# FRBNY-DSGE/SMC.jl

Measured on AMD Instinct MI355X. Metric: particle-stages/sec, higher is better.
Workload: dtype f64; 1 GPU; gauss10_isotropic_adaptive_phi_n100k (BASELINE config 2); n_parts_total=100000, n_parts_per_gpu=100000, n_para=10, n_phi=300, resampling=systematic, n_blocks=1, n_mh_steps=1, launch_mode=direct, history=True, parallelism=particles sharded x1

## Files before the change

smc.jl_amd/csrc/prof2.hpp:

```cpp
#pragma once

static int prof2_report(smcmi_handle *h0, const Geo2 &g0, int seg_launches) {
    {
        long long pr[128], gt[64], gp[64];
        HIP_TRY(hipMemcpy(pr, h0->e2->d_prof + PROF2_SEG0, 64 * sizeof(long long), hipMemcpyDeviceToHost));
        HIP_TRY(hipMemcpy(gt, h0->e2->d_prof + PROF2_GATH, sizeof(gt), hipMemcpyDeviceToHost));
        HIP_TRY(hipMemcpy(gp, h0->e2->d_prof + PROF2_GPOLL, sizeof(gp), hipMemcpyDeviceToHost));
        if (seg_launches > 0) {
            fprintf(stderr, "[smcmi3] stage %d worker 0 ticks: correction + row %lld | wait for the totals %lld | decision + proposal %lld | MH steps %lld | mutation row %lld | next stage's draws %lld | wait for the totals %lld | begin %lld | stage %lld\n",
                    h0->e2->prof_stage, pr[2] - pr[1], pr[3] - pr[2], pr[4] - pr[3], pr[5] - pr[4], pr[6] - pr[5], pr[7] - pr[6], pr[8] - pr[7], pr[9] - pr[8], pr[9] - pr[1]);
            fprintf(stderr, "[smcmi3]   stamps relative to the stage's first:");
            for (int q = 1; q <= 9; ++q) fprintf(stderr, " [%d] %lld", q, pr[q] - pr[1]);
            fprintf(stderr, "\n");
            {
                long long sp[10];
                HIP_TRY(hipMemcpy(sp, h0->e2->d_prof + PROF2_SEL, sizeof(sp), hipMemcpyDeviceToHost));
                if (sp[9]) fprintf(stderr, "[smcmi3]   selection inside the segment (wall clock, us): particle stored %.2f | chunk offsets %.2f | scan + cum %.2f | stores acknowledged %.2f | hand-over %.2f | chunk ends %.2f | search %.2f | rows gathered %.2f | moment row %.2f | hand-over %.2f\n",
                                   0.0, (sp[1] - sp[0]) * 0.01, (sp[2] - sp[1]) * 0.01, (sp[3] - sp[2]) * 0.01, (sp[4] - sp[3]) * 0.01, (sp[5] - sp[4]) * 0.01, (sp[6] - sp[5]) * 0.01, (sp[7] - sp[6]) * 0.01, (sp[8] - sp[7]) * 0.01, (sp[9] - sp[8]) * 0.01);
            }
            fprintf(stderr, "[smcmi3]   decision + proposal: totals -> covariance, shuffle %lld | block matrices %lld | Cholesky + log det %lld | rest %lld\n",
                    pr[30] - pr[3], pr[31] - pr[30], pr[32] - pr[31], pr[4] - pr[32]);
        }
        if (seg_launches > 0) {
            const int Wk = g0.Vl * g0.nb2;
            std::vector<long long> ws(4 * (size_t)Wk);
            HIP_TRY(hipMemcpy(ws.data(), h0->e2->d_prof + PROF2_WORK, sizeof(long long) * ws.size(), hipMemcpyDeviceToHost));
            for (int kind = 0; kind < 2; ++kind) {
                long long p_min = 0, p_max = 0, s_min = 0, s_max = 0;
                for (int b = 0; b < Wk; ++b) {
                    const long long pb = ws[4 * b + 2 * kind], sb = ws[4 * b + 2 * kind + 1];
                    if (!b || pb < p_min) p_min = pb;
                    if (!b || pb > p_max) p_max = pb;
                    if (!b || sb < s_min) s_min = sb;
                    if (!b || sb > s_max) s_max = sb;
                }
                fprintf(stderr, "[smcmi3] hand-over %d (%s rows): rows published over %.2f us (worker 0 at +%.2f); totals seen by the first worker +%.2f, the last +%.2f, worker 0 +%.2f after the first row\n",
                        kind, kind ? "mutation" : "correction", (p_max - p_min) * 0.01, (ws[2 * kind] - p_min) * 0.01, (s_min - p_min) * 0.01, (s_max - p_min) * 0.01, (ws[2 * kind + 1] - p_min) * 0.01);
                for (int v = 0; v < g0.Vl; ++v) {
                    long long lastrow = 0;
                    for (int b = v; b < Wk; b += g0.Vl) lastrow = std::max(lastrow, ws[4 * b + 2 * kind]);
                    fprintf(stderr, "[smcmi3]   gatherer %d: its last row +%.2f | first words seen +%.2f | %lld sweep(s) done +%.2f | totals posted +%.2f (started waiting at +%.2f)\n", v, (lastrow - p_min) * 0.01,
                            (gp[4 * v + 2 * kind] - p_min) * 0.01, gp[4 * v + 2 * kind + 1],
                            (gt[6 * v + 3 * kind + 1] - p_min) * 0.01, (gt[6 * v + 3 * kind + 2] - p_min) * 0.01, (gt[6 * v + 3 * kind] - p_min) * 0.01);
                }
            }
        }
        if (!g0.direct && !g0.inker && !g0.wide) {
            std::vector<long long> cs(3 * PROF2_BLOCKS);
            HIP_TRY(hipMemcpy(cs.data(), h0->e2->d_prof + PROF2_CENSUS, sizeof(long long) * cs.size(), hipMemcpyDeviceToHost));
            long long t_min = 0, t_max = 0, sum = 0;
            int nbk = 0;
            std::map<long long, std::vector<std::pair<long long, int>>> per_cu;
            for (int b = 0; b < PROF2_BLOCKS; ++b) {
                const long long t_a = cs[3 * b], t_b = cs[3 * b + 1];
                if (!t_a || !t_b) continue;
                if (!nbk || t_a < t_min) t_min = t_a;
                if (!nbk || t_b > t_max) t_max = t_b;
                sum += t_b - t_a;
                ++nbk;
                per_cu[cs[3 * b + 2]].push_back({t_a, +1});
                per_cu[cs[3 * b + 2]].push_back({t_b, -1});
            }
            int hist[9] = {0, 0, 0, 0, 0, 0, 0, 0, 0};
            for (auto &kv : per_cu) {
                std::sort(kv.second.begin(), kv.second.end());
                int cur = 0, mx = 0;
                for (auto &ev : kv.second) { cur += ev.second; mx = std::max(mx, cur); }
                hist[std::min(mx, 8)] += 1;
            }
            if (nbk) {
                fprintf(stderr, "[smcmi2] K2b census: %d blocks on %d CUs, first start -> last end %.2f us, mean block %.2f us, mean residency %.1f blocks; CUs by the most blocks they held at once:", nbk,
                        (int)per_cu.size(), (t_max - t_min) * 0.01, sum * 0.01 / nbk, (double)sum / (double)std::max<long long>(1, t_max - t_min));
                for (int k = 1; k <= 8; ++k) if (hist[k]) fprintf(stderr, " %d x %d", hist[k], k);
                int st_h[8] = {0, 0, 0, 0, 0, 0, 0, 0}, du_h[8] = {0, 0, 0, 0, 0, 0, 0, 0};
                const double st_e[7] = {1, 2, 5, 10, 15, 20, 25}, du_e[7] = {8, 12, 16, 20, 24, 28, 32};
                for (int b = 0; b < PROF2_BLOCKS; ++b) {
                    if (!cs[3 * b] || !cs[3 * b + 1]) continue;
                    const double st = (cs[3 * b] - t_min) * 0.01, du = (cs[3 * b + 1] - cs[3 * b]) * 0.01;
                    int k = 0; while (k < 7 && st >= st_e[k]) ++k; st_h[k] += 1;
                    k = 0; while (k < 7 && du >= du_e[k]) ++k; du_h[k] += 1;
                }
                fprintf(stderr, "\n[smcmi2]   started at <1 <2 <5 <10 <15 <20 <25 >=25 us:");
                for (int k = 0; k < 8; ++k) fprintf(stderr, " %d", st_h[k]);
                fprintf(stderr, "; ran <8 <12 <16 <20 <24 <28 <32 >=32 us:");
                for (int k = 0; k < 8; ++k) fprintf(stderr, " %d", du_h[k]);
                fprintf(stderr, "\n");
            }
        }
        HIP_TRY(hipMemcpy(pr, h0->e2->d_prof + PROF2_K1, 128 * sizeof(long long), hipMemcpyDeviceToHost));
        for (int blk = 0; blk < 2; ++blk) {
            fprintf(stderr, "[smcmi2] K1 %s block ticks:", blk ? "mid" : "0");
            for (int q = 1; q <= 5; ++q) fprintf(stderr, " %lld", pr[blk * 32 + q] - pr[blk * 32 + q - 1]);
            fprintf(stderr, "  total %lld\n[smcmi2] K2 %s block ticks:", pr[blk * 32 + 5] - pr[blk * 32], blk ? "mid" : "0");
            for (int q = 1; q <= 11; ++q) fprintf(stderr, " %lld", pr[64 + blk * 32 + q] - pr[64 + blk * 32 + q - 1]);
            fprintf(stderr, "  total %lld\n", pr[64 + blk * 32 + 10] - pr[64 + blk * 32]);
        }
    }
    return 0;
}
```

smc.jl_amd/csrc/stage2.hpp:

```cpp
#pragma once
#include "kernels.hpp"

namespace smcmi {

constexpr int RMAX_IDX = 32;
constexpr int T1 = 512;

constexpr int PROF2_BLOCKS = 4096;
constexpr int PROF2_K1 = 0, PROF2_K2 = 64, PROF2_CENSUS = 128, PROF2_SEG0 = PROF2_CENSUS + 3 * PROF2_BLOCKS, PROF2_SEL = PROF2_SEG0 + 64,
              PROF2_GATH = PROF2_SEL + 16, PROF2_GPOLL = PROF2_GATH + 64, PROF2_WORK = PROF2_GPOLL + 64, PROF2_WORDS = PROF2_WORK + 4 * 256;
#define K2_STAMP(prof, slot)                                                                                                   \
    do {                                                                                                                      \
        if ((prof) != nullptr && threadIdx.x == 0 && (blockIdx.x == 0 || blockIdx.x == gridDim.x / 2)) {                       \
            unsigned long long tt_;                                                                                           \
            asm volatile("s_waitcnt vmcnt(0) lgkmcnt(0)\n\ts_memtime %0\n\ts_waitcnt lgkmcnt(0)" : "=s"(tt_)::"memory");       \
            (prof)[(blockIdx.x == 0 ? 0 : 32) + (slot)] = (long long)tt_;                                                      \
        }                                                                                                                     \
    } while (0)

#define K3_STAMP_ANY(prof, slot)                                                                                               \
    do {                                                                                                                      \
        if ((prof) != nullptr && threadIdx.x == 0) {                                                                           \
            unsigned long long tt_;                                                                                           \
            asm volatile("s_waitcnt vmcnt(0) lgkmcnt(0)\n\ts_memtime %0\n\ts_waitcnt lgkmcnt(0)" : "=s"(tt_)::"memory");       \
            (prof)[(slot)] = (long long)tt_;                                                                                   \
        }                                                                                                                     \
    } while (0)

struct Geo2 {
    long long N, n, nv;
    int V, Vl, v0;
    int nb1, nb2, nbg;
    long long per1, perg;
    int t2;
    int direct;
    int inker;
    int wide;
};

struct Rows2 {
    const double *p;
    int nvs, nr, ld;
    const unsigned long long *mb;
    unsigned tag;
    unsigned long long *to;
};

constexpr int MB_LD = 72;
constexpr int MB_TABLE_WORDS = V2_MAXV * MB_LD * 2;
constexpr int MB_KINDS = 2;
constexpr int MB_WORDS = MB_KINDS * 2 * MB_TABLE_WORDS;
constexpr long long MB_TIMEOUT_TICKS_DEFAULT = 1000000000ll;
constexpr int MB_FLAG_WORDS = 2;
constexpr int MB_SEG_OFF = MB_WORDS + MB_FLAG_WORDS;
constexpr int MB_SEG_KIND_WORDS = V2_MAXV * MB_LD * 2;
constexpr int MB_SEG_COPY_WORDS = 2 * MB_SEG_KIND_WORDS;
constexpr int MB_ALLOC_WORDS = MB_SEG_OFF + 2 * MB_SEG_COPY_WORDS;
constexpr long long MB_SEL_CS_WORDS = 1024 * 2, MB_SEL_T_WORDS = V2_MAXV * 2 * 2, MB_SEL_GM_WORDS = V2_MAXV * 72 * 2;
constexpr long long MB_SEL_OFF = MB_ALLOC_WORDS, MB_SEL_TABLE_WORDS = MB_SEL_CS_WORDS + MB_SEL_T_WORDS + MB_SEL_GM_WORDS;
__device__ inline void mb_store(unsigned long long *w, double v, unsigned tag) {
    const unsigned long long b = (unsigned long long)__double_as_longlong(v);
    __hip_atomic_store(w, ((unsigned long long)tag << 32) | (b & 0xffffffffull), __ATOMIC_RELAXED, __HIP_MEMORY_SCOPE_SYSTEM);
    __hip_atomic_store(w + 1, ((unsigned long long)tag << 32) | (b >> 32), __ATOMIC_RELAXED, __HIP_MEMORY_SCOPE_SYSTEM);
}
__device__ inline double mb_load(const unsigned long long *w, unsigned tag, unsigned long long *to) {
    unsigned long long a = __hip_atomic_load(w, __ATOMIC_RELAXED, __HIP_MEMORY_SCOPE_SYSTEM);
    unsigned long long b = __hip_atomic_load(w + 1, __ATOMIC_RELAXED, __HIP_MEMORY_SCOPE_SYSTEM);
    if ((unsigned)(a >> 32) != tag || (unsigned)(b >> 32) != tag) {
        const long long t0 = wall_clock64();
        do {
            if (__hip_atomic_load(to, __ATOMIC_RELAXED, __HIP_MEMORY_SCOPE_AGENT)) return __builtin_nan("");
            __builtin_amdgcn_s_sleep(2);
            a = __hip_atomic_load(w, __ATOMIC_RELAXED, __HIP_MEMORY_SCOPE_SYSTEM);
            b = __hip_atomic_load(w + 1, __ATOMIC_RELAXED, __HIP_MEMORY_SCOPE_SYSTEM);
            if (wall_clock64() - t0 > (long long)__hip_atomic_load(to + 1, __ATOMIC_RELAXED, __HIP_MEMORY_SCOPE_AGENT)) {
                __hip_atomic_store(to, 1ull, __ATOMIC_RELAXED, __HIP_MEMORY_SCOPE_AGENT);
                return __builtin_nan("");
            }
        } while ((unsigned)(a >> 32) != tag || (unsigned)(b >> 32) != tag);
    }
    return __longlong_as_double((long long)((b << 32) | (a & 0xffffffffull)));
}
template <int M, int T>
__device__ inline void mbox_totals(const Rows2 &R, double *vt, double *tot, int max_idx) {
    for (int idx = threadIdx.x; idx < R.nvs * M; idx += T) {
        const int v = idx / M, k = idx % M;
        vt[idx] = mb_load(R.mb + ((long long)v * MB_LD + k) * 2, R.tag, R.to);
    }
    __syncthreads();
    for (int k = threadIdx.x; k < M; k += T) {
        const bool mx = k == max_idx;
        double t = mx ? -__builtin_inf() : 0.0;
        for (int v = 0; v < R.nvs; ++v) { const double x = vt[v * M + k]; t = mx ? fmax(t, x) : t + x; }
        tot[k] = t;
    }
    __syncthreads();
}

struct Begin2 {
    int stage, final, spec, j;
    double phi_prev, phi_n, phi_prop, ess_bar, gprime, pred_delta;
    double accept;
    double e_shift, e_center;
    double cfac;
    double e_seen;
};
struct Post2 {
    int stage, j, resampled_last, do_resample, resamples, fold_valid;
    double phi_n, phi_prop, ess, sumw, sumw2, logz, c, accept, e_center, e_shift;
    double e_seen;
// ... 1182 lines not shown
    const double *wt;
    double *rows_mut;
    Tail2 tail;
    double *hist_W;
    long long hist_ld;
    Records rec;
    int debug;
    long long *prof;
};

__device__ inline void post2(int n, const Begin2 &bg, const Post2 &po, const RunParams &rp, double s1, double s2, double ess, int rs, Post2 *out) {
    const double a = bg.accept;
    Post2 p = po;
    p.stage = n; p.j = bg.j; p.resampled_last = rs; p.do_resample = rs; p.resamples = po.resamples + rs; p.fold_valid = 1;
    p.phi_n = bg.phi_n; p.phi_prop = bg.phi_prop; p.ess = ess; p.sumw = s1; p.sumw2 = s2;
    const double dlz = (bg.phi_n - bg.phi_prev) * bg.e_shift;
    p.logz = po.logz + (log(s1 / (double)rp.n_parts) + dlz);
    p.c = po.c * bg.cfac;
    p.accept = a; p.e_center = bg.e_center; p.e_shift = bg.e_shift; p.e_seen = bg.e_seen;
    *out = p;
}

struct Prop2 {
    double *covl, *A, *mean;
    int *bfree, *bptr, *fi;
    double *Lraw, *logdet, *mub, *sdd, *sdn;
    int *ball, *loff;
    double *Ls;
};
template <int DB>
__device__ inline bool chol_full(double (&r)[12], int lane) {
    double q[DB];
#pragma unroll
    for (int k = 0; k < DB; ++k) q[k] = r[k];
    const bool ok = chol_rows_in_regs<DB, true, true>(q, DB, lane);
#pragma unroll
    for (int k = 0; k < DB; ++k) r[k] = q[k];
    return ok;
}
__device__ inline bool chol_full_dispatch(double (&r)[12], int d, int lane) {
    switch (d) {
    case 2: return chol_full<2>(r, lane); case 3: return chol_full<3>(r, lane); case 4: return chol_full<4>(r, lane);
    case 5: return chol_full<5>(r, lane); case 6: return chol_full<6>(r, lane); case 7: return chol_full<7>(r, lane);
    case 8: return chol_full<8>(r, lane); case 9: return chol_full<9>(r, lane); default: return chol_full<10>(r, lane);
    }
}

__device__ inline int shuffle_partner(unsigned long long seed, unsigned stage, int i0, int nf) {
    int jx = 0;
    if (i0 >= 1 && i0 < nf) {
        double ua, ub;
        uniform_pair(seed, 0ull, stage, rng_tag(P_BLK, (unsigned)i0, 0), ua, ub);
        jx = (int)(ua * (double)(i0 + 1));
        if (jx > i0) jx = i0;
    }
    return jx;
}

__device__ inline void shuffle_trace(int jx, int lane, int nf, int nb, int *bfree, int *bptr) {
    int pos = lane;
    for (int i = 1; i < nf; ++i) {
        const int ji = __shfl(jx, i, 64);
        pos = pos == i ? ji : (pos == ji ? i : pos);
    }
    if (lane < nf) bfree[lane] = pos;
    const int sub = (nf + nb - 1) / nb;
    if (lane < nb) bptr[lane] = lane * sub;
    if (lane == nb) bptr[nb] = nf;
}

constexpr int A1F_SHUF = 1;
constexpr int A1F_NOMIX = 2;
constexpr int A1F_LOGDET = 4;
constexpr int A1F_LS = 8;
#ifndef SMCMI_A1FAST
#define SMCMI_A1FAST (A1F_SHUF | A1F_NOMIX | A1F_LOGDET | A1F_LS)
#endif
constexpr int A1F_BOUNDS = 16;
constexpr int A1F_PRIOR = 32;
#ifndef SMCMI_A1TARGET
#define SMCMI_A1TARGET (A1F_BOUNDS | A1F_PRIOR)
#endif
static_assert(A1F_BOUNDS == (TGT_BOUNDS << 4) && A1F_PRIOR == (TGT_PRIOR << 4), "k2_mh_steps hands FAST >> 4 to mh_step");

template <int CHM = 12, int FAST = 0>
__device__ inline bool proposal2(const double *T, const double *shift, int d, int nf, int nb, double c, unsigned long long seed,
                                 unsigned stage, const Prop2 &P, int *s_fail, int TT, int jx_pre, long long *prof = nullptr, long long *prof_any = nullptr) {
    const int t = threadIdx.x, da = d + 1;
    const double sw = T[0];
    if (t == 0) *s_fail = 0;
    for (int e = t; e < d * d; e += TT) {
        int a = e / d, b = e % d;
        if (a > b) { const int tmp = a; a = b; b = tmp; }
        const int ra = a + 1, rb = b + 1;
        const int p = ra * da - ra * (ra - 1) / 2 + (rb - ra);
        P.covl[e] = T[p] / sw - (T[a + 1] / sw) * (T[b + 1] / sw);
    }
    for (int a = t; a < d; a += TT) P.mean[a] = shift[a] + T[a + 1] / sw;
    if constexpr (!(FAST & A1F_SHUF)) {
        if (t >= 64 && t < 128) shuffle_trace(jx_pre, t - 64, nf, nb, P.bfree, P.bptr);
    }
    if constexpr ((FAST & A1F_LS) != 0) { if (nb == 1) for (int e = t; e < d * d; e += TT) P.Ls[e] = 0.0; }
    __syncthreads();
    K2_STAMP(prof, 4);
    K3_STAMP_ANY(prof_any, 0);
    auto sig = [&](int f, int g2) { const int a = P.fi[f], b = P.fi[g2]; return (P.covl[a * d + b] + P.covl[b * d + a]) / 2.0; };
    for (int i = t; i < nf; i += TT) {
        const int f = P.bfree[i];
        [[maybe_unused]] const double sff = sig(f, f);
        P.ball[i] = P.fi[f];
        if constexpr (!(FAST & A1F_NOMIX)) {
            P.mub[i] = P.mean[P.fi[f]];
            P.sdd[i] = sqrt(c * c * sff);
            P.sdn[i] = sqrt(sff);
        }
    }
    {
        const int sub = (nf + nb - 1) / nb;
        for (int e = t; e < nf * nf; e += TT) {
            int b = 0, rem = e;
            while (b < nb - 1 && rem >= sub * sub) { rem -= sub * sub; ++b; }
            const int p0 = P.bptr[b], db = P.bptr[b + 1] - p0;
            if (rem < db * db) P.A[b * sub * sub + rem] = c * c * sig(P.bfree[p0 + rem / db], P.bfree[p0 + rem % db]);
        }
    }
    __syncthreads();
    K2_STAMP(prof, 5);
    K3_STAMP_ANY(prof_any, 1);
    {
        const int sub = (nf + nb - 1) / nb, wave = t >> 6, lane = t & 63, nwv = TT >> 6;
        for (int b = wave; b < nb; b += nwv) {
            const int p0 = P.bptr[b], db = P.bptr[b + 1] - p0, off = b * sub * sub;
            double r[CHM];
#pragma unroll
            for (int k = 0; k < CHM; ++k) r[k] = (lane < db && k < db) ? P.A[off + lane * db + k] : 0.0;
            bool ok;
            if constexpr (CHM == 12) {
                if (db == d && d <= 10 && d >= 2) ok = chol_full_dispatch(r, d, lane);
                else ok = chol_rows_in_regs<12, true>(r, db, lane);
            } else ok = chol_rows_in_regs<CHM, true>(r, db, lane);
            if (!ok && lane == 0) *s_fail = 1;
            if constexpr ((FAST & A1F_LS) != 0) {
                if (nb == 1) {
                    const int col = lane < db ? P.ball[lane] : 0;
#pragma unroll
                    for (int k = 0; k < CHM; ++k)
                        if (lane < db && k <= lane) P.Ls[k * d + col] = r[k];
                }
            }
#pragma unroll
            for (int k = 0; k < CHM; ++k)
                if (lane < db && k < db) P.Lraw[off + lane * db + k] = k <= lane ? r[k] : 0.0;
            if constexpr ((FAST & A1F_LOGDET) != 0) {
                if (lane == 0) P.loff[b] = off;
            } else {
                double dg = 1.0;
#pragma unroll
                for (int k = 0; k < CHM; ++k) dg = (k == lane) ? r[k] : dg;
                const double lg = (lane < db) ? log(dg) : 0.0;
                double ld = 0.0;
#pragma unroll
                for (int i = 0; i < CHM; ++i)
                    if (i < db) ld += bcast_lane(lg, i);
                if (lane == 0) { P.logdet[b] = 2.0 * ld; P.loff[b] = off; }
            }
        }
    }
    __syncthreads();
    K2_STAMP(prof, 6);
    K3_STAMP_ANY(prof_any, 2);
    return *s_fail == 0;
}

template <int D>
struct Mut2Lds : MutBodyLds<D> {
    static constexpr int DA = D + 1, NP = DA * (DA + 1) / 2, NPF = NP + 2;
    double *s_vt, *s_tot, *covl, *sig_f, *Aw, *Lw, *mean_s, *mu_f;
    int *bfree, *fi, *fi_j;
    __device__ explicit Mut2Lds(double *sm, bool lik_data = true) {
        if (lik_data) place<LIK_LDS_CAP>(sm); else place<0>(sm);
    }
    template <int CAP>
    __device__ void place(double *sm) {
        using namespace lds;
        constexpr Mut2Layout O = mut2(D, 8, CAP);
        this->template place_body<8, CAP>(sm);
        s_vt = lds_at<double, O[M_svt]>(sm); s_tot = lds_at<double, O[M_stot]>(sm);
        covl = lds_at<double, O[M_covl]>(sm); sig_f = lds_at<double, O[M_sigf]>(sm); Aw = lds_at<double, O[M_Aw]>(sm); Lw = lds_at<double, O[M_Lw]>(sm);
        mean_s = lds_at<double, O[M_mean]>(sm); mu_f = lds_at<double, O[M_muf]>(sm);
        bfree = lds_at<int, O[M_bfree]>(sm); fi = lds_at<int, O[M_fi]>(sm); fi_j = lds_at<int, O[M_fij]>(sm);
    }
};

struct Mut2Stage {
    Begin2 bg;
    Post2 po;
    int fail;
};

template <int D, int T>
__device__ inline bool k2_prologue(DevState *st, Ctl2 *ctl, const ModelDev *md, const Mut2Args &ma, const Mut2Lds<D> &L, Mut2Stage *S, int nb, int nf,
                                   int *rs_out, int writer_ov = -1, bool own_cfac = false) {
    constexpr int NP = Mut2Lds<D>::NP, NPF = Mut2Lds<D>::NPF;
    const int tid = threadIdx.x, n = ma.n;
    const bool writer = writer_ov >= 0 ? writer_ov != 0 : blockIdx.x == 0;
    constexpr int NWB = sizeof(Begin2) / sizeof(double), NWP = sizeof(Post2) / sizeof(double);
    if (tid < NWB) reinterpret_cast<double *>(&S->bg)[tid] = reinterpret_cast<const double *>(&ctl->bg)[tid];
    if (tid < NWP) reinterpret_cast<double *>(&S->po)[tid] = reinterpret_cast<const double *>(&ctl->ps[(n - 1) & 1])[tid];
    const double thr = st->rp.threshold, rtol = st->rp.phi_rtol;
    for (int k = tid; k < D; k += T) {
        L.m_lo[k] = md->lo[k]; L.m_hi[k] = md->hi[k]; L.m_a[k] = md->prior_a[k]; L.m_b[k] = md->prior_b[k]; L.m_k[k] = md->prior_k[k];
        L.m_fix[k] = md->fixed[k]; L.m_fam[k] = md->prior_family[k];
    }
    for (int k = tid; k < 2 * LIK_PAR_MAX; k += T) L.l_par[k] = md->lik[k / LIK_PAR_MAX].par[k % LIK_PAR_MAX];
    if (tid < nf) L.fi[tid] = md->free_inds[tid];
    const int jx_pre = (tid >= 64 && tid < 128) ? shuffle_partner(ma.seed, (unsigned)n, tid - 64, nf) : 0;
    K2_STAMP(ma.prof, 1);
    if (ma.cmrows.mb) {
        __syncthreads();
        if (S->bg.stage != n || !S->bg.final || S->po.stage != n - 1) return false;
    }
    reduce_rows<pad2(NPF), 1, T>(ma.cmrows, L.s_vt, L.s_tot);
    K2_STAMP(ma.prof, 2);
    if (S->bg.stage != n || !S->bg.final || S->po.stage != n - 1) return false;
    if (own_cfac) {
        if (tid == 0) { const double a = S->bg.accept, tg = st->rp.target; S->bg.cfac = 0.95 + 0.10 * exp(16.0 * (a - tg)) / (1.0 + exp(16.0 * (a - tg))); }
        __syncthreads();
    }
    double ess;
    const int dec = decide2(S->bg, thr, rtol, L.s_tot[0], L.s_tot[1], &ess);
    const bool stall = dec == 4 || dec < 0 || (dec == 1 && !ma.sel_enqueued);
    if (stall) {
        if (writer && tid == 0) {
            if (dec < 0) { ma.rec.phi[n - 1] = S->bg.phi_n; ma.rec.ess[n - 1] = ess; ctl->status.err = dec; }
            ctl->status.stage = n;
            ctl->status.code = dec == 4 ? 4 : (dec < 0 ? 9 : 3);
        }
        return false;
    }
    const int rs = dec == 1 ? 1 : 0;
    *rs_out = rs;
    K2_STAMP(ma.prof, 3);
    if (rs) reduce_rows<pad2(NP), 1, T>(ma.gmrows, L.s_vt, L.s_tot + 2);
    Prop2 P{L.covl, L.Aw, L.mean_s, L.bfree, L.bptr_s, L.fi, L.Lraw, L.logdet_s, L.mub_raw, L.sdd_raw, L.sdn_raw, L.ball_raw, L.loff_s};
    if (!proposal2<(D > 12 ? 16 : 12)>(L.s_tot + 2, S->po.shift, D, nf, nb, S->po.c * S->bg.cfac, ma.seed, (unsigned)n, P, &S->fail, T, jx_pre, ma.prof)) {
        if (writer && tid == 0) { ctl->status.err = SMCMI_ERR_POSDEF; ctl->status.stage = n; ctl->status.code = 9; }
        return false;
    }
    K2_STAMP(ma.prof, 7);
    return true;
}

// ... 305 lines not shown
```

smc.jl_amd/csrc/stage3.hpp:

```cpp
#pragma once
#include "stage2.hpp"

namespace smcmi {

#ifndef SMCMI_K3_WAVES
#define SMCMI_K3_WAVES 2
#endif
constexpr int TICK3_STRIDE = 32;
constexpr int SEG3_TICKS = (V2_MAXV + 1) * TICK3_STRIDE;

struct RecA3 {
    int act, pad;
    Begin2 bg;
};
template <int D>
struct Prop3 {
    double Lraw[D * D], logdet[D], mub[D], sdd[D], sdn[D];
    int ball[D + (D & 1)], bptr[D + 2 + (D & 1)], loff[D + (D & 1)];
};
template <int D>
struct RecB3 {
    int act, pad;
    Post2 po;
    Prop3<D> pr;
// ... 930 lines not shown
__device__ inline bool k3_rides(const RunParams &rp, const Seg3Args &sa, const Post2 &po, int n, bool sys) {
    (void)sys;
    return rp.use_fixed_schedule && rp.shift_lag && n < sa.n_last && po.phi_n < 1.0 && !(rp.stop_stage > 0 && n >= rp.stop_stage) && n + 1 <= rp.max_stages;
}

#define K3_DO_DRAW(ns)                                                                                                                          \
    do {                                                                                                                                        \
        if ((ns) <= sa.n_last) k3_draw_park<D, !ALPHA1>(z_park, ma.seed, pid_park, (unsigned)(ns), db0);                               \
        K3_STAMP(sa.prof, 7);                                                                                                                   \
    } while (0)
#define K3_DO_BEGIN(ns, po_p, pair, ACT)                                                                                                         \
    do {                                                                                                                                        \
        const unsigned tag_p_ = sa.tag_base | (unsigned)((ns) - 1);                                                                             \
        bool ok_;                                                                                                                               \
        if (RIDE && (pair)) {                                                                                                                   \
            const unsigned tag_c_ = sa.tag_base | (unsigned)(ns);                                                                               \
            ok_ = rows_two ? gather_totals_pair<2>(sa.g_mut + K3_RPAR((ns) - 1), tag_p_, sa.g_cm + K3_RPAR(ns), MCM, tag_c_, g.V, sa.to, &s_to, s_totm, s_tot, s_vt)  \
                           : gather_totals_pair(rows_direct ? sa.g_mut + K3_RPAR((ns) - 1) : sa.gt_mut + K3_TPAR((ns) - 1), tag_p_,             \
                                                rows_direct ? sa.g_cm + K3_RPAR(ns) : sa.gt_cm + K3_TPAR(ns), MCM, tag_c_, g.V, sa.to, &s_to, s_totm, s_tot, s_vt, sys,  \
                                                (writer && sys) ? sa.vt_mut_out : nullptr);                                                     \
        } else {                                                                                                                                \
            ok_ = rows_two ? gather_totals<2>(sa.g_mut + K3_RPAR((ns) - 1), g.V, RMUT, RMAX_IDX, tag_p_, sa.to, &s_to, s_tot, s_vt)            \
                           : K3_TOTALS_MUT(rows_direct ? sa.g_mut + K3_RPAR((ns) - 1) : sa.gt_mut + K3_TPAR((ns) - 1), tag_p_,                 \
                                           (writer && sys) ? sa.vt_mut_out : nullptr);                                                          \
        }                                                                                                                                       \
        if (!ok_) { timed_out = true; ACT = -1; break; }                                                                                        \
        K3_STAMP(sa.prof, 8);                                                                                                                   \
        K3_WALL(sa.gprof, PROF2_WORK + 4 * blockIdx.x + 3);                                                                                            \
        ACT = begin_stage((ns), (po_p), (RIDE && (pair)) ? s_totm : s_tot);                                                                     \
        constexpr int NWB_ = sizeof(Begin2) / sizeof(double);                                                                                   \
        if (ACT == 0 && writer && tid < NWB_) reinterpret_cast<double *>(&ctl->bg)[tid] = reinterpret_cast<const double *>(&s_a.bg)[tid];       \
        K3_STAMP(sa.prof, 9);                                                                                                                   \
    } while (0)
#if (K3HO) & K3H_FETCH
#define K3_TOTALS_CM(tbl_, tag_) k3_totals<MCM, -1, 0>(&s_ho, (tag_))
#define K3_TOTALS_MUT(tbl_, tag_, out_) k3_totals<RMUT, RMAX_IDX, 1>(&s_ho, (tag_))
#else
#define K3_TOTALS_CM(tbl_, tag_) gather_totals((tbl_), g.V, MCM, -1, (tag_), sa.to, &s_to, s_tot, s_vt, sys)
#define K3_TOTALS_MUT(tbl_, tag_, out_) gather_totals((tbl_), g.V, RMUT, RMAX_IDX, (tag_), sa.to, &s_to, s_tot, s_vt, sys, (out_))
#endif
#define K3_GATHER(M_, MAXI_, KIND_, tag_) \
    (__builtin_expect(g.nb2 <= K3G_ROWS, 1) ? k3_gather<M_, MAXI_, KIND_>(&s_gh, (tag_)) : k3_gather_wide<M_, MAXI_, KIND_>(&s_gh, (tag_)))
#if (K3HO) & K3H_SW
#define K3_FILL_SW(po_n_)                                                                                                                       \
    do {                                                                                                                                        \
        if (tid < 64) {                                                                                                                         \
            const int jj_ = (po_n_).j - 1 + tid;                                                                                                \
            s_sw[tid] = (!rp.use_fixed_schedule && jj_ >= 0 && jj_ < rp.n_phi) ? sa.sched[jj_] : 2.0;                                           \
        }                                                                                                                                       \
    } while (0)
#else
#define K3_FILL_SW(po_n_) (void)0
#endif
#define K3_RPAR(stage) ((RIDE && ((stage) & 1)) ? (long long)k3_copy_words(g.Vl * g.nb2) : 0)
#define K3_TPAR(stage) ((RIDE && ((stage) & 1)) ? (sys ? (long long)MB_SEG_COPY_WORDS : (long long)k3_copy_words(g.Vl * g.nb2)) : 0)
#ifdef SMCMI_K3_CH2
#define K3_SWAP_CHUNKS()                                                                                                                        \
    do {                                                                                                                                        \
        if constexpr (CH > 1) {                                                                                                                 \
            double *s2_ = st2 + tid;                                                                                                            \
            _Pragma("unroll") for (int k_ = 0; k_ < D; ++k_) { const double t_ = s2_[k_ * T3]; s2_[k_ * T3] = x[k_]; x[k_] = t_; }              \
            { double t_; t_ = s2_[D * T3]; s2_[D * T3] = like; like = t_; t_ = s2_[(D + 1) * T3]; s2_[(D + 1) * T3] = lprior; lprior = t_;      \
              t_ = s2_[(D + 2) * T3]; s2_[(D + 2) * T3] = like_prev; like_prev = t_; t_ = s2_[(D + 3) * T3]; s2_[(D + 3) * T3] = acc_val; acc_val = t_; \
              t_ = s2_[(D + 4) * T3]; s2_[(D + 4) * T3] = Wt; Wt = t_; t_ = s2_[(D + 5) * T3]; s2_[(D + 5) * T3] = v; v = t_; }                \
            cur ^= 1;                                                                                                                           \
            beg = beg_c[cur]; end = end_c[cur]; i = beg + tid; live = i < end; has = has_c[cur]; rowi = rowi_c[cur];                            \
            pid = (unsigned long long)(ma.gid0 + i);                                                                                            \
        }                                                                                                                                       \
    } while (0)
#define K3_HAS has
#define K3_CHUNKS_BEGIN for (int it = 0; it < CH; ++it) {
#define K3_CHUNKS_END if (it + 1 < CH) K3_SWAP_CHUNKS(); }
#define K3_PARKED_DRAWS (cur == 0)
#define K3_V_RESET() v = 0.0
#else
#define K3_HAS true
#define K3_CHUNKS_BEGIN {
#define K3_CHUNKS_END }
#define K3_PARKED_DRAWS true
#define K3_V_RESET() (void)0
#endif

constexpr int k3_fast_bits(bool alpha1, bool ride, int ch, bool sys) {
    return alpha1 ? ((SMCMI_A1FAST) | ((!ride && ch == 1 && !sys) ? (SMCMI_A1TARGET) : 0)) : 0;
}
template <int D, bool ALPHA1, bool RIDE, int CH = 1, bool SYS = false>
__global__ void __launch_bounds__(T3, SMCMI_K3_WAVES) k3_segment(CloudPtrs cl, DevState *st, Ctl2 *ctl, const ModelDev *md, Geo2 g, Mut2Args ma, Seg3Args sa, int nb, int nf) {
    constexpr int NPF = Mut2Lds<D>::NPF, MCM = pad2(NPF);
    extern __shared__ __attribute__((aligned(16))) double sm[];
    __shared__ RecA3 s_a;
    __shared__ RecB3<D> s_b[2];
    __shared__ double s_vt[V2_MAXV * RMUT * 4], s_tot[pad2(NPF) > RMUT ? pad2(NPF) : RMUT], s_sw[64];
    __shared__ double s_totm[RIDE ? RMUT : 2];
    static_assert(V2_MAXV * RMUT * 4 >= V2_MAXV * (72 + RMUT), "gather_totals_pair stages both tables in s_vt");
    __shared__ double red[(T3 / 64) * (cm_row_ld(NPF) > 64 ? cm_row_ld(NPF) : 64)];
    __shared__ int s_act, s_to, s_fail;
    __shared__ double s_cfac;
#ifdef SMCMI_K3_CH2
    __shared__ Sel2Geo s_ch2[2];
#endif
    __shared__ RunParams s_rp;
    __shared__ double mixbuf[ALPHA1 ? 1 : MixDense<D>::DOUBLES + D * D];
    __shared__ int mixpos[ALPHA1 ? 1 : D];
    __shared__ double mixzt[ALPHA1 ? 1 : T3 * D];
    Mut2Lds<D> L(sm);
    constexpr lds::Seg3Layout O3 = k3_layout(D, ALPHA1, CH);
    const int tid = threadIdx.x;
    constexpr int FAST = k3_fast_bits(ALPHA1, RIDE, CH, SYS);
#ifdef SMCMI_K3_CH2
    const int W = g.Vl * ((g.nb2 + CH - 1) / CH);
#else
    static_assert(CH == 1, "two chunks per worker: a translation unit that defines SMCMI_K3_CH2 (inst3.hip -DSMCMI_INST3_C=2)");
    const int W = g.Vl * g.nb2;
#endif
    const bool worker = (int)blockIdx.x < W, writer = blockIdx.x == 0;
    if (tid == 0) { s_rp = st->rp; s_to = 0; }
#if (K3HO) & K3H_FETCH
    __shared__ K3Ho s_ho;
    if (tid == 64) {
        const bool direct = g.nb2 == 1;
        s_ho.tbl[0] = direct ? sa.g_cm : sa.gt_cm; s_ho.tbl[1] = direct ? sa.g_mut : sa.gt_mut;
        s_ho.to = sa.to; s_ho.tot = (K3_LDS double *)s_tot; s_ho.vt = (K3_LDS double *)s_vt; s_ho.s_to = (K3_LDS int *)&s_to; s_ho.nvs = g.V;
    }
#endif
#if (K3HO) & K3H_GATHER
    __shared__ K3Gh s_gh;
    if (tid == 65 && !worker) {
        const int vg_ = (int)blockIdx.x - W;
        s_gh.tbl[0] = sa.g_cm + (long long)vg_ * g.nb2 * MCM * 2; s_gh.tbl[1] = sa.g_mut + (long long)vg_ * g.nb2 * RMUT * 2;
        s_gh.dst[0] = sa.gt_cm + (long long)(g.v0 + vg_) * MCM * 2; s_gh.dst[1] = sa.gt_mut + (long long)(g.v0 + vg_) * RMUT * 2;
        s_gh.to = sa.to; s_gh.pw = sa.gprof ? sa.gprof + PROF2_GPOLL + 4 * vg_ : nullptr; s_gh.ptag = sa.tag_base | (unsigned)sa.prof_stage;
        s_gh.stage = (K3_LDS double *)lds_at<double, O3[lds::S_gather]>(sm); s_gh.s_to = (K3_LDS int *)&s_to; s_gh.nr = g.nb2;
    }
#endif
    if (tid < nf) L.fi[tid] = md->free_inds[tid];
    __syncthreads();
    const RunParams &rp = s_rp;
    int n = sa.n_first;
    int rs0 = 0;
    if (!sa.enter_mut) {
        const int act = begin2_block<T3>(n, st, ctl, sa.mrows, 1, sa.sched, ma.rec, &s_b[(n - 1) & 1].po, &s_a.bg, s_vt, s_tot, s_sw, &s_act);
        if (act != 0) { k3_leave_note(sa, ctl); return; }
        if (tid == 0) {
            const double a = s_a.bg.accept, tg = rp.target;
            s_cfac = 0.95 + 0.10 * exp(16.0 * (a - tg)) / (1.0 + exp(16.0 * (a - tg)));
            s_a.bg.cfac = s_cfac;
        }
        __syncthreads();
    } else {
        constexpr int NWB = sizeof(Begin2) / sizeof(double), NWP = sizeof(Post2) / sizeof(double), NPm = Mut2Lds<D>::NP;
        if (tid < NWB) reinterpret_cast<double *>(&s_a.bg)[tid] = reinterpret_cast<const double *>(&ctl->bg)[tid];
        if (tid < NWP) reinterpret_cast<double *>(&s_b[(n - 1) & 1].po)[tid] = reinterpret_cast<const double *>(&ctl->ps[(n - 1) & 1])[tid];
        if (ma.cmrows.mb) {
            __syncthreads();
            if (s_a.bg.stage != n || !s_a.bg.final || s_b[(n - 1) & 1].po.stage != n - 1) { k3_leave_note(sa, ctl); return; }
        }
        reduce_rows<MCM, 1, T3>(ma.cmrows, s_vt, s_tot);
        if (s_a.bg.stage != n || !s_a.bg.final || s_b[(n - 1) & 1].po.stage != n - 1) { k3_leave_note(sa, ctl); return; }
        double ess;
        const int dec = decide2(s_a.bg, rp.threshold, rp.phi_rtol, s_tot[0], s_tot[1], &ess);
        if (dec == 4 || dec < 0 || (dec == 1 && !ma.sel_enqueued)) {
            if (writer && tid == 0) {
                if (dec < 0) { ma.rec.phi[n - 1] = s_a.bg.phi_n; ma.rec.ess[n - 1] = ess; ctl->status.err = dec; }
                ctl->status.stage = n;
                ctl->status.code = dec == 4 ? 4 : (dec < 0 ? 9 : 3);
            }
            k3_leave_note(sa, ctl);
// ... 197 lines not shown
        for (int k = tid; k < D; k += T3) m_rb[k] = md->prior_rb[k];
        mv.rb = m_rb;
    }
    LikView lv[2];
    stage_lik(ma.lik[0], ma.lik[1], L.l_par, L.l_dat, T3, lv);
    const int db0 = nb == 1 ? nf : (nf + nb - 1) / nb;
    k3_draw_park<D, !ALPHA1>(z_park, ma.seed, pid_park, (unsigned)n, db0);
    __syncthreads();
    int done = 0;
    bool timed_out = false;
    const bool rows_direct = g.nb2 == 1 && !sys;
    const bool rows_two = g.nb2 == 2 && !sys;
    bool rides = false;
#ifdef SMCMI_K3_CH2
    double v = v_entered;
#endif
    for (;; ++n) {
        K3_STAMP(sa.prof, 1);
        RecB3<D> &B = s_b[n & 1];
        const Post2 &po = s_b[(n - 1) & 1].po;
        const unsigned tag = sa.tag_base | (unsigned)n;
        L.Lraw = B.pr.Lraw; L.logdet_s = B.pr.logdet; L.mub_raw = B.pr.mub; L.sdd_raw = B.pr.sdd; L.sdn_raw = B.pr.sdn;
        L.ball_raw = B.pr.ball; L.bptr_s = B.pr.bptr; L.loff_s = B.pr.loff;
        const bool first = n == sa.n_first;
        const bool entered = sa.enter_mut && first;
        int rs = entered ? rs0 : 0;
#ifndef SMCMI_K3_CH2
        double v = entered ? v_entered : 0.0;
#endif
        int act = 0;
        if (!entered && !(RIDE && !first && !rides)) {
            const double phi = rides ? (n <= rp.n_phi ? sa.sched[n - 1] : 1.0) : s_a.bg.phi_n, phi_prev = rides ? po.phi_n : s_a.bg.phi_prev;
            const double esh = rides ? po.e_seen - (rp.shift_lag == n ? 1e6 : (rp.shift_lag == -n ? -1e6 : 0.0)) : s_a.bg.e_shift;
            K3_CHUNKS_BEGIN
            unsigned long long *my_cm = sa.g_cm + K3_RPAR(n) + (long long)rowi * MCM * 2;
            K3_V_RESET();
            if constexpr (ALPHA1) {
                double xx[D + 1];
#pragma unroll
                for (int a = 0; a <= D; ++a) xx[a] = 0.0;
                if (K3_LIVE) {
                    double inc;
                    v = k2_cm_weight<D>([&](int a) { return x[a]; }, po.shift, like, like_prev, Wt, esh, phi, phi_prev, pw, logp_old, xx, &inc);
                    if (hist) {
                        const double unshift = exp((phi - phi_prev) * esh);
                        sa.hist_w[(long long)(n - 1) * sa.hist_ld + i] = inc * unshift;
                    }
                }
                k2_cm_row_one<D, T3 / 64, ((K3HO) & K3H_DEAD) != 0>(v, xx, K3_LIVE, red, [&](int idx, double val) { if (K3_HAS) gran_store(my_cm + idx * 2, val, tag); });
            } else {
                constexpr int NCH = (NPF + 63) / 64;
                double acc[NCH * 64];
#pragma unroll
                for (int q = 0; q < NCH * 64; ++q) acc[q] = 0.0;
                if (K3_LIVE) {
                    double inc;
                    v = k2_cm_particle<D>(acc, [&](int a) { return x[a]; }, po.shift, like, like_prev, Wt, esh, phi, phi_prev, pw, logp_old, &inc);
                    if (hist) {
                        const double unshift = exp((phi - phi_prev) * esh);
                        sa.hist_w[(long long)(n - 1) * sa.hist_ld + i] = inc * unshift;
                    }
                }
                k2_cm_row_f<D>(acc, red, [&](int idx, double val) { if (K3_HAS) gran_store(my_cm + idx * 2, val, tag); });
            }
            if (K3_HAS && tid >= NPF && tid < MCM) gran_store(my_cm + tid * 2, 0.0, tag);
            K3_CHUNKS_END
        }
        K3_STAMP(sa.prof, 2);
        K3_WALL(sa.gprof, PROF2_WORK + 4 * blockIdx.x + 0);
        if constexpr (RIDE) {
            if (!first) {
                K3_DO_DRAW(n);
                K3_DO_BEGIN(n, po, rides, act);
                if (act == 0 && !rides) {
                    if (writer && tid == 0) { ctl->status.err = SMCMI_ERR_STATE; ctl->status.stage = n; ctl->status.code = 9; __hip_atomic_store(sa.to, 2ull, __ATOMIC_RELAXED, __HIP_MEMORY_SCOPE_AGENT); }
                    act = -1;
                }
            }
        }
        if (act != 0) break;
        const double e_center = s_a.bg.e_center;
        const int jx_pre = (tid >= 64 && tid < 128) ? shuffle_partner(ma.seed, (unsigned)n, tid - 64, nf) : 0;
        if constexpr ((FAST & A1F_SHUF) != 0) { if (tid >= 64 && tid < 128) shuffle_trace(jx_pre, tid - 64, nf, nb, L.bfree, L.bptr_s); }
        if (!entered && !(RIDE && rides) && !(rows_two ? gather_totals<2>(sa.g_cm + K3_RPAR(n), g.V, MCM, -1, tag, sa.to, &s_to, s_tot, s_vt)
                                   : K3_TOTALS_CM(rows_direct ? sa.g_cm + K3_RPAR(n) : sa.gt_cm + K3_TPAR(n), tag))) { timed_out = true; break; }
        K3_STAMP(sa.prof, 3);
        K3_WALL(sa.gprof, PROF2_WORK + 4 * blockIdx.x + 1);
        double ess = s_tot[0] * s_tot[0] / s_tot[1];
        int dec = entered ? 0 : decide2(s_a.bg, rp.threshold, rp.phi_rtol, s_tot[0], s_tot[1], &ess);
#ifndef SMCMI_K3_CH2
        if (__builtin_expect(dec == 1 && sa.sel != nullptr, 0)) {
            double *sto = lds_at<double, O3[lds::S_cols]>(sm);
            if constexpr (k3_sel_cols(D, ALPHA1) == 0) sto = sa.sel->transit + (long long)blockIdx.x * (D + 5) * T3;
            double *stx = sto + 5 * T3;
            __syncthreads();
            sto[tid] = v;
#pragma unroll
            for (int k = 0; k < D; ++k) stx[k * T3 + tid] = x[k];
            sto[T3 + tid] = like; sto[2 * T3 + tid] = lprior; sto[3 * T3 + tid] = like_prev; sto[4 * T3 + tid] = acc_val;
#if (K3HO) & K3H_REDRAW
            const int bad = k3_select_inside<D, !ALPHA1>(sa.sel, cl.buf[0], cl.n, cl.R, g.N, g.V * g.nb1, g.V, rowi, i, beg, end, tag, n, ma.seed, ma.gid0, sa.g_cm + K3_RPAR(n), sa.to, &s_to, s_tot, s_vt, s_sw,
                                                red, z_park, stx, sto, po.shift, (sa.prof && writer && n == sa.prof_stage) ? sa.gprof + PROF2_SEL : nullptr, rows_direct, rows_two, db0);
#else
            const int bad = k3_select_inside<D>(sa.sel, cl.buf[0], cl.n, cl.R, g.N, g.V * g.nb1, g.V, rowi, i, beg, end, tag, n, ma.seed, ma.gid0, sa.g_cm + K3_RPAR(n), sa.to, &s_to, s_tot, s_vt, s_sw,
                                                red, z_park, stx, sto, po.shift, (sa.prof && writer && n == sa.prof_stage) ? sa.gprof + PROF2_SEL : nullptr, rows_direct, rows_two);
#endif
            if (bad) { timed_out = true; break; }
#pragma unroll
            for (int k = 0; k < D; ++k) x[k] = stx[k * T3 + tid];
            like = sto[T3 + tid]; lprior = sto[2 * T3 + tid]; like_prev = sto[3 * T3 + tid]; acc_val = sto[4 * T3 + tid];
#if !((K3HO) & K3H_REDRAW)
            k3_draw_park<D, !ALPHA1>(z_park, ma.seed, pid, (unsigned)n, db0);
#endif
            __syncthreads();
            rs = 1; dec = 0;
        }
#else
        if (__builtin_expect(dec == 1 && sa.sel != nullptr, 0)) {
            double *tr = sa.sel->transit + (long long)blockIdx.x * (D + 5) * T3;
            __syncthreads();
            tr[tid] = v;
#pragma unroll
            for (int k = 0; k < D; ++k) tr[(5 + k) * T3 + tid] = x[k];
            tr[T3 + tid] = like; tr[2 * T3 + tid] = lprior; tr[3 * T3 + tid] = like_prev; tr[4 * T3 + tid] = acc_val;
            const int bad = k3_select_two<D>(sa.sel, cl.buf[0], cl.n, cl.R, g.N, g.V * g.nb1, g.V, s_ch2, cur, tr, st2, tag, n, ma.seed, ma.gid0, sa.g_cm + K3_RPAR(n), sa.to, &s_to, s_tot, s_vt, s_sw,
                                             red, z_park, po.shift);
            if (bad) { timed_out = true; break; }
#pragma unroll
            for (int k = 0; k < D; ++k) x[k] = tr[(5 + k) * T3 + tid];
            like = tr[T3 + tid]; lprior = tr[2 * T3 + tid]; like_prev = tr[3 * T3 + tid]; acc_val = tr[4 * T3 + tid];
            k3_draw_park<D, !ALPHA1>(z_park, ma.seed, pid_park, (unsigned)n, db0);
            __syncthreads();
            rs = 1; dec = 0;
        }
#endif
        if (dec != 0) {
            if (writer && tid == 0) {
                if (dec < 0) { ma.rec.phi[n - 1] = s_a.bg.phi_n; ma.rec.ess[n - 1] = ess; ctl->status.err = dec; }
                ctl->status.stage = n;
                ctl->status.code = dec < 0 ? 9 : (dec == 4 ? 4 : 6);
            }
            break;
        }
        if (tid == T3 - 64) post2(n, s_a.bg, po, rp, s_tot[0], s_tot[1], ess, rs, &B.po);
        {
            Prop2 P{L.covl, L.Aw, L.mean_s, L.bfree, L.bptr_s, L.fi, L.Lraw, L.logdet_s, L.mub_raw, L.sdd_raw, L.sdn_raw, L.ball_raw, L.loff_s, L.Ls};
            if (!proposal2<12, FAST>(s_tot + 2, po.shift, D, nf, nb, po.c * s_a.bg.cfac, ma.seed, (unsigned)n, P, &s_fail, T3, jx_pre, nullptr,
                           (sa.prof && writer && n == sa.prof_stage) ? sa.prof + 30 : nullptr)) {
                if (writer && tid == 0) {
                    ctl->status.err = SMCMI_ERR_POSDEF; ctl->status.stage = n; ctl->status.code = 9;
                    __hip_atomic_store(sa.to, 2ull, __ATOMIC_RELAXED, __HIP_MEMORY_SCOPE_AGENT);
                }
                break;
            }
        }
        if (tid < D) B.po.shift[tid] = L.mean_s[tid];
        __syncthreads();
        if (writer) {
            if (tid == 0) { ma.rec.phi[n - 1] = B.po.phi_n; ma.rec.ess[n - 1] = B.po.ess; ma.rec.resampled[n - 1] = rs; ma.rec.c[n - 1] = B.po.c; }
            if (tid < D) st->mean[tid] = L.mean_s[tid];
            for (int e = tid; e < D * D; e += T3) st->cov[e] = L.covl[e];
            constexpr int NWP = sizeof(Post2) / sizeof(double);
            if (tid < NWP) reinterpret_cast<double *>(&ctl->ps[n & 1])[tid] = reinterpret_cast<const double *>(&B.po)[tid];
        }
        K3_STAMP(sa.prof, 4);
        const double phi_n = B.po.phi_n, nrm_sumw = B.po.sumw;
        K3_CHUNKS_BEGIN
        double accept = 0.0;
        double step_prob, uc, z[D];
        if (K3_PARKED_DRAWS) {
            const double *p = z_park + tid;
            step_prob = p[0];
            uc = p[T3];
#pragma unroll
            for (int e = 0; e < D; ++e) z[e] = p[(2 + e) * T3];
        } else mh_draw<D>(ma.seed, pid, (unsigned)n, 0u, db0, step_prob, uc, z);
        if (K3_LIVE) {
            Wt = rs ? 1.0 : (v * nrm_N) / nrm_sumw;
            if (ma.hist_W && ma.store_history) ma.hist_W[(long long)(n - 1) * ma.hist_ld + i] = Wt;
        }
        k2_mh_steps<D, ALPHA1, T3, true, false, FAST>(L, mixbuf, mixpos, mixzt, ma, g.n, lv, mv, nb, nf, K3_LIVE, i, pid, (unsigned)n, phi_n, x, like, lprior, like_prev, accept,
                                         step_prob, uc, z);
        if (K3_LIVE) acc_val = accept / (double)nf;
        K3_STAMP(sa.prof, 5);
        {
            double *plain = ma.rows_mut + (long long)rowi * RMUT;
            unsigned long long *my_mut = sa.g_mut + K3_RPAR(n) + (long long)rowi * RMUT * 2;
            K3_LIVE_ROW_DECL;
            k2_mut_row_f<T3>(ma.adaptive != 0, like, like_prev, K3_LIVE_ROW ? Wt : 0.0, K3_LIVE_ROW ? acc_val : 0.0, e_center, K3_LIVE_ROW, rs != 0, red, L.red,
                             [&](int idx, double val) { if (K3_HAS) { gran_store(my_mut + idx * 2, val, tag); plain[idx] = val; } },
                             energy_base(like_prev, rp.pw, rp.logp_old));
            if (K3_HAS && tid == RMUT - 1) gran_store(my_mut + tid * 2, 0.0, tag);
        }
        K3_CHUNKS_END
        ++done;
        K3_STAMP(sa.prof, 6);
        K3_WALL(sa.gprof, PROF2_WORK + 4 * blockIdx.x + 2);
        if constexpr (RIDE) rides = k3_rides(rp, sa, B.po, n, sys);
        else {
            K3_FILL_SW(B.po);
            K3_DO_DRAW(n + 1);
            K3_DO_BEGIN(n + 1, B.po, false, act);
            if (act != 0) break;
        }
    }
#undef K3_RPAR
#undef K3_LIVE
#undef K3_LIVE_ROW_DECL
#undef K3_LIVE_ROW
#undef K3_FILL_SW
#undef K3_TOTALS_CM
#undef K3_TOTALS_MUT
#undef K3_TPAR
#undef K3_DO_DRAW
#undef K3_DO_BEGIN
#undef K3_SWAP_CHUNKS
#undef K3_HAS
#undef K3_CHUNKS_BEGIN
#undef K3_CHUNKS_END
#undef K3_PARKED_DRAWS
#undef K3_V_RESET
    if (live && !timed_out) {
#pragma unroll
        for (int k = 0; k < D; ++k) col(cl, 0, k)[i] = x[k];
        col(cl, 0, D)[i] = like; col(cl, 0, D + 1)[i] = lprior; col(cl, 0, D + 2)[i] = like_prev;
        col(cl, 0, D + 3)[i] = acc_val; col(cl, 0, D + 4)[i] = Wt;
    }
#ifdef SMCMI_K3_CH2
    {
        const long long io = beg_c[cur ^ 1] + tid;
        if (io < end_c[cur ^ 1] && !timed_out) {
// ... 15 lines not shown
```

Before: 3.777 billion particle-stages/s.

## Fuse single-block proposal covariance build and Cholesky into one wave pass

Adds a fused proposal path for the single-block case. Wave 0 builds the covariance block in registers directly from the weighted totals using lane broadcasts, then factors it, while other waves compute the full covariance and mean in parallel. The ball index setup and Ls zeroing move ahead of the totals wait, so they overlap with it. This is meant to drop the intermediate LDS matrix writes and the barriers on the serial per-stage proposal path, at the cost of extra code complexity and compile-time variants.

```diff
diff --git a/smc.jl_amd/csrc/prof2.hpp b/smc.jl_amd/csrc/prof2.hpp
--- a/smc.jl_amd/csrc/prof2.hpp
+++ b/smc.jl_amd/csrc/prof2.hpp
@@ -20,6 +20,10 @@
             }
             fprintf(stderr, "[smcmi3]   decision + proposal: totals -> covariance, shuffle %lld | block matrices %lld | Cholesky + log det %lld | rest %lld\n",
                     pr[30] - pr[3], pr[31] - pr[30], pr[32] - pr[31], pr[4] - pr[32]);
+#ifdef SMCMI_PROF_CHOL
+            fprintf(stderr, "[smcmi3]   proposal stamps after the totals: decision [35] %lld | [30] %lld | [31] %lld | [33] %lld | [34] %lld | [32] %lld | [4] %lld\n",
+                    pr[35] - pr[3], pr[30] - pr[3], pr[31] - pr[3], pr[33] - pr[3], pr[34] - pr[3], pr[32] - pr[3], pr[4] - pr[3]);
+#endif
         }
         if (seg_launches > 0) {
             const int Wk = g0.Vl * g0.nb2;
diff --git a/smc.jl_amd/csrc/stage2.hpp b/smc.jl_amd/csrc/stage2.hpp
--- a/smc.jl_amd/csrc/stage2.hpp
+++ b/smc.jl_amd/csrc/stage2.hpp
@@ -26,6 +26,12 @@
             (prof)[(slot)] = (long long)tt_;                                                                                   \
         }                                                                                                                     \
     } while (0)
+
+#ifdef SMCMI_PROF_CHOL
+#define K3_STAMP_FUSED(prof, slot) K3_STAMP_ANY(prof, slot)
+#else
+#define K3_STAMP_FUSED(prof, slot) do { } while (0)
+#endif
 
 struct Geo2 {
     long long N, n, nv;
@@ -1374,12 +1380,20 @@
 #define SMCMI_A1TARGET (A1F_BOUNDS | A1F_PRIOR)
 #endif
 static_assert(A1F_BOUNDS == (TGT_BOUNDS << 4) && A1F_PRIOR == (TGT_PRIOR << 4), "k2_mh_steps hands FAST >> 4 to mh_step");
+constexpr int A1F_FUSE = 64;
+#ifndef SMCMI_A1FUSE
+#define SMCMI_A1FUSE A1F_FUSE
+#endif
+#ifndef SMCMI_FUSE_VARIANT
+#define SMCMI_FUSE_VARIANT 0
+#endif
 
 template <int CHM = 12, int FAST = 0>
 __device__ inline bool proposal2(const double *T, const double *shift, int d, int nf, int nb, double c, unsigned long long seed,
                                  unsigned stage, const Prop2 &P, int *s_fail, int TT, int jx_pre, long long *prof = nullptr, long long *prof_any = nullptr) {
     const int t = threadIdx.x, da = d + 1;
     const double sw = T[0];
+    [[maybe_unused]] const bool PRE = (FAST & A1F_FUSE) != 0 && nb == 1;
     if (t == 0) *s_fail = 0;
     for (int e = t; e < d * d; e += TT) {
         int a = e / d, b = e % d;
@@ -1392,7 +1406,7 @@
     if constexpr (!(FAST & A1F_SHUF)) {
         if (t >= 64 && t < 128) shuffle_trace(jx_pre, t - 64, nf, nb, P.bfree, P.bptr);
     }
-    if constexpr ((FAST & A1F_LS) != 0) { if (nb == 1) for (int e = t; e < d * d; e += TT) P.Ls[e] = 0.0; }
+    if constexpr ((FAST & A1F_LS) != 0) { if (nb == 1 && !PRE) for (int e = t; e < d * d; e += TT) P.Ls[e] = 0.0; }
     __syncthreads();
     K2_STAMP(prof, 4);
     K3_STAMP_ANY(prof_any, 0);
@@ -1400,7 +1414,7 @@
     for (int i = t; i < nf; i += TT) {
         const int f = P.bfree[i];
         [[maybe_unused]] const double sff = sig(f, f);
-        P.ball[i] = P.fi[f];
+        if (!PRE) P.ball[i] = P.fi[f];
         if constexpr (!(FAST & A1F_NOMIX)) {
             P.mub[i] = P.mean[P.fi[f]];
             P.sdd[i] = sqrt(c * c * sff);
@@ -1426,11 +1440,13 @@
             double r[CHM];
 #pragma unroll
             for (int k = 0; k < CHM; ++k) r[k] = (lane < db && k < db) ? P.A[off + lane * db + k] : 0.0;
+            K3_STAMP_FUSED(prof_any, 3);
             bool ok;
             if constexpr (CHM == 12) {
                 if (db == d && d <= 10 && d >= 2) ok = chol_full_dispatch(r, d, lane);
                 else ok = chol_rows_in_regs<12, true>(r, db, lane);
             } else ok = chol_rows_in_regs<CHM, true>(r, db, lane);
+            K3_STAMP_FUSED(prof_any, 4);
             if (!ok && lane == 0) *s_fail = 1;
             if constexpr ((FAST & A1F_LS) != 0) {
                 if (nb == 1) {
@@ -1460,6 +1476,70 @@
     }
     __syncthreads();
     K2_STAMP(prof, 6);
+    K3_STAMP_ANY(prof_any, 2);
+    return *s_fail == 0;
+}
+
+template <int CHM, int DMAX>
+__device__ inline bool proposal2_fused(const double *T, const double *shift, int d, int nf, double c, const Prop2 &P, int *s_fail, int TT,
+                                       bool unpublished, long long *prof_any = nullptr) {
+    int t = threadIdx.x;
+    asm volatile("" : "+v"(t));
+    const int da = d + 1;
+    const double sw = T[0];
+#if (SMCMI_FUSE_VARIANT) & 2
+    if (t >= 64 && t < 64 + nf) P.ball[t - 64] = P.fi[P.bfree[t - 64]];
+    for (int e = t; e < d * d; e += TT) P.Ls[e] = 0.0;
+    __syncthreads();
+#else
+    if (unpublished) __syncthreads();
+#endif
+    if (t < 64) {
+        const int lane = t, db = nf;
+        if (t == 0) *s_fail = 0;
+        const int a = lane < nf ? P.ball[lane] : 0;
+        const double ma = T[a + 1] / sw;
+        double r[CHM];
+#pragma unroll
+        for (int k = 0; k < CHM; ++k) {
+            r[k] = 0.0;
+            if (k < DMAX) {
+                const int b = __builtin_amdgcn_readlane(a, k);
+                const double mb = bcast_lane(ma, k);
+                const bool swap = a > b;
+                const int ra = (swap ? b : a) + 1, rb = (swap ? a : b) + 1;
+                const int p = ra * da - ra * (ra - 1) / 2 + (rb - ra);
+                const double v = T[p] / sw - (swap ? mb : ma) * (swap ? ma : mb);
+                r[k] = (lane < nf && k < nf) ? c * c * ((v + v) / 2.0) : 0.0;
+            }
+        }
+        K3_STAMP_FUSED(prof_any, 0);
+        bool ok;
+        if constexpr (CHM == 12) {
+            if (db == d && d <= 10 && d >= 2) ok = chol_full_dispatch(r, d, lane);
+            else ok = chol_rows_in_regs<12, true>(r, db, lane);
+        } else ok = chol_rows_in_regs<CHM, true>(r, db, lane);
+        K3_STAMP_FUSED(prof_any, 1);
+        if (!ok && lane == 0) *s_fail = 1;
+#pragma unroll
+        for (int k = 0; k < CHM; ++k)
+            if (lane < db && k <= lane) P.Ls[k * d + a] = r[k];
+#pragma unroll
+        for (int k = 0; k < CHM; ++k)
+            if (lane < db && k < db) P.Lraw[lane * db + k] = k <= lane ? r[k] : 0.0;
+        if (lane == 0) P.loff[0] = 0;
+    } else if (t < TT - 64) {
+        const int TC = TT - 128;
+        for (int e = t - 64; e < d * d; e += TC) {
+            int a = e / d, b = e % d;
+            if (a > b) { const int tmp = a; a = b; b = tmp; }
+            const int ra = a + 1, rb = b + 1;
+            const int p = ra * da - ra * (ra - 1) / 2 + (rb - ra);
+            P.covl[e] = T[p] / sw - (T[a + 1] / sw) * (T[b + 1] / sw);
+        }
+        for (int a = t - 64; a < d; a += TC) P.mean[a] = shift[a] + T[a + 1] / sw;
+    }
+    __syncthreads();
     K3_STAMP_ANY(prof_any, 2);
     return *s_fail == 0;
 }
diff --git a/smc.jl_amd/csrc/stage3.hpp b/smc.jl_amd/csrc/stage3.hpp
--- a/smc.jl_amd/csrc/stage3.hpp
+++ b/smc.jl_amd/csrc/stage3.hpp
@@ -1036,7 +1036,7 @@
 #endif
 
 constexpr int k3_fast_bits(bool alpha1, bool ride, int ch, bool sys) {
-    return alpha1 ? ((SMCMI_A1FAST) | ((!ride && ch == 1 && !sys) ? (SMCMI_A1TARGET) : 0)) : 0;
+    return alpha1 ? ((SMCMI_A1FAST) | ((!ride && ch == 1 && !sys) ? ((SMCMI_A1TARGET) | (SMCMI_A1FUSE)) : 0)) : 0;
 }
 template <int D, bool ALPHA1, bool RIDE, int CH = 1, bool SYS = false>
 __global__ void __launch_bounds__(T3, SMCMI_K3_WAVES) k3_segment(CloudPtrs cl, DevState *st, Ctl2 *ctl, const ModelDev *md, Geo2 g, Mut2Args ma, Seg3Args sa, int nb, int nf) {
@@ -1400,12 +1400,23 @@
         const double e_center = s_a.bg.e_center;
         const int jx_pre = (tid >= 64 && tid < 128) ? shuffle_partner(ma.seed, (unsigned)n, tid - 64, nf) : 0;
         if constexpr ((FAST & A1F_SHUF) != 0) { if (tid >= 64 && tid < 128) shuffle_trace(jx_pre, tid - 64, nf, nb, L.bfree, L.bptr_s); }
+#if !((SMCMI_FUSE_VARIANT) & 2)
+        if constexpr ((FAST & A1F_FUSE) != 0) {
+            if (nb == 1) {
+                int t_ = tid;
+                asm volatile("" : "+v"(t_));
+                if (t_ >= 64 && t_ < 64 + nf) L.ball_raw[t_ - 64] = L.fi[L.bfree[t_ - 64]];
+                for (int e = t_; e < D * D; e += T3) L.Ls[e] = 0.0;
+            }
+        }
+#endif
         if (!entered && !(RIDE && rides) && !(rows_two ? gather_totals<2>(sa.g_cm + K3_RPAR(n), g.V, MCM, -1, tag, sa.to, &s_to, s_tot, s_vt)
                                    : K3_TOTALS_CM(rows_direct ? sa.g_cm + K3_RPAR(n) : sa.gt_cm + K3_TPAR(n), tag))) { timed_out = true; break; }
         K3_STAMP(sa.prof, 3);
         K3_WALL(sa.gprof, PROF2_WORK + 4 * blockIdx.x + 1);
         double ess = s_tot[0] * s_tot[0] / s_tot[1];
         int dec = entered ? 0 : decide2(s_a.bg, rp.threshold, rp.phi_rtol, s_tot[0], s_tot[1], &ess);
+        K3_STAMP_FUSED((sa.prof && writer && n == sa.prof_stage) ? sa.prof + 30 : nullptr, 5);
 #ifndef SMCMI_K3_CH2
         if (__builtin_expect(dec == 1 && sa.sel != nullptr, 0)) {
             double *sto = lds_at<double, O3[lds::S_cols]>(sm);
@@ -1463,8 +1474,11 @@
         if (tid == T3 - 64) post2(n, s_a.bg, po, rp, s_tot[0], s_tot[1], ess, rs, &B.po);
         {
             Prop2 P{L.covl, L.Aw, L.mean_s, L.bfree, L.bptr_s, L.fi, L.Lraw, L.logdet_s, L.mub_raw, L.sdd_raw, L.sdn_raw, L.ball_raw, L.loff_s, L.Ls};
-            if (!proposal2<12, FAST>(s_tot + 2, po.shift, D, nf, nb, po.c * s_a.bg.cfac, ma.seed, (unsigned)n, P, &s_fail, T3, jx_pre, nullptr,
-                           (sa.prof && writer && n == sa.prof_stage) ? sa.prof + 30 : nullptr)) {
+            if (!(((FAST & A1F_FUSE) != 0 && nb == 1 && !((SMCMI_FUSE_VARIANT) & 8))
+                      ? proposal2_fused<12, D>(s_tot + 2, po.shift, D, nf, po.c * s_a.bg.cfac, P, &s_fail, T3, entered,
+                                               (sa.prof && writer && n == sa.prof_stage) ? sa.prof + 30 : nullptr)
+                      : proposal2<12, FAST>(s_tot + 2, po.shift, D, nf, nb, po.c * s_a.bg.cfac, ma.seed, (unsigned)n, P, &s_fail, T3, jx_pre, nullptr,
+                           (sa.prof && writer && n == sa.prof_stage) ? sa.prof + 30 : nullptr))) {
                 if (writer && tid == 0) {
                     ctl->status.err = SMCMI_ERR_POSDEF; ctl->status.stage = n; ctl->status.code = 9;
                     __hip_atomic_store(sa.to, 2ull, __ATOMIC_RELAXED, __HIP_MEMORY_SCOPE_AGENT);
```

Measured after the change: 3.861 billion particle-stages/s (median of 6 runs). +2.2%, better.
